# yml-bit/CTA-GAN

Measured on AMD Instinct MI355X. Metric: paired 512x512 slices/sec (G+D step); generator rel-L2 vs CPU reference, higher is better.
Workload: dtype bf16; 1 GPU; HdGan stage-2 full G+D train step (G, Reg, STN, D_m, losses, Adam x3), 16 paired 512x512 slices/GPU; per_gpu_batch=16, global_batch=16, size=512, parallelism=single, rccl_ranks=1, dp_backend=none

## Files before the change

### cta_gan_amd/csrc/conv_wgrad.hip

```cpp
#include <stdlib.h>
#include "conv_dispatch.h"

struct WgradArgs {
    const void* g;
    const void* x;
    float* part;
    int B, Hs, Ws, Mc, g_ld;
    int Hi, Wi, Nc, x_ld;
    int is, pad_mode;
    int slab, sps;
    int ntaps;
    int taps[64];
};

template <typename T> struct WgCfg;
template <> struct WgCfg<bf16_t> { static constexpr int PK = 64, PK_MT = 32, PADB = 32; };
template <> struct WgCfg<float> { static constexpr int PK = 32, PK_MT = 16, PADB = 64; };

template <typename T, int BM, int BN, int NT>
__global__ __launch_bounds__(256) void conv_wgrad_kernel(const WgradArgs a) {
    constexpr int EPC = VecOf<T>::N;
    constexpr int PK = NT > 1 ? WgCfg<T>::PK_MT : WgCfg<T>::PK;
    constexpr int RSM = BM * (int)sizeof(T) + WgCfg<T>::PADB;
    constexpr int RSN = BN * (int)sizeof(T) + WgCfg<T>::PADB;
// ... 899 lines not shown
                h.tmap[cnt++] = t;
            }
            if (cnt == 0) continue;
            const int kh = win.kh(), kw = win.kw();
            ok = cnt == kh * kw;
            for (int i = 0; ok && i < cnt; ++i) {
                const int tw = a.taps[h.tmap[i]];
                const int qy = (tap_dy(tw) - py) / 2, qx = (tap_dx(tw) - px) / 2;
                ok = (qy == win.dy0() + i / kw) && (qx == win.dx0() + i % kw);
            }
            h.g = g; h.x = x; h.part = part;
            h.B = B; h.Hs = Hs; h.Ws = Ws; h.Mc = Mc; h.g_ld = g_ld;
            h.Hi = Hi; h.Wi = Wi; h.Nc = Nc; h.x_ld = x_ld;
            h.pad_mode = pad_mode; h.sps = a.sps; h.ntaps = cnt; h.gtaps = ntaps;
            h.kw = kw; h.khb = kh; h.dy0 = win.dy0(); h.dx0 = win.dx0();
            h.is = 2; h.py = py; h.px = px;
            h.phases = pair ? 3 : 1; h.g_lo = g_ld / 2; h.x_lo = x_ld / 2; h.phase_split = split;
            h.no_reuse = ctg_knobs().wg_no_reuse;
            h.prefetch = !ctg_knobs().wg_noprefetch;
            h.xcd = !ctg_knobs().wg_noxcd;
            const int bm = h.Mc % 64 == 0 ? 64 : h.Mc % 32 == 0 ? 32 : 16, bn = h.Nc % 64 == 0 ? 64 : 32;
            ok = ok && bm >= 32 && !(bm == 32 && bn == 32) && (cnt == 1 || cnt == 2 || cnt == 4) && kw <= 2 && kh <= 2;
            covered += cnt;
            ++nph;
        }
        if (ok && covered == ntaps && ntaps == 9 && nph == 4 && !split) {
            if (taps_3x3(a.taps, false)) {
                WgHaloArgs h = ph[0];
                h.ntaps = 9; h.gtaps = 9; h.kw = 2; h.khb = 2; h.dy0 = -1; h.dx0 = -1; h.py = 0; h.px = 0;
                const int rc = launch_wg_s2m(h, st);
                if (rc != -1) return rc;
            }
        }
        if (ok && covered == ntaps) {
            for (int p = 0; p < nph; ++p) {
                const int rc = launch_wgh_any(ph[p], st);
                if (rc != 0) return rc == -1 ? CTG_EINVAL : rc;
            }
            return split ? 3 : 0;
        }
    }
    if (pair) return 2;
    if (Mc % 32) return CTG_EINVAL;
    return dtype == DT_BF16 ? launch_wg_t<bf16_t>(a, st) : launch_wg_t<float>(a, st);
}

#define RED_MAX_T 24
struct ReduceList {
    const float* part[RED_MAX_T];
    float* dst[RED_MAX_T];
    long sm[RED_MAX_T], sn[RED_MAX_T], stp[RED_MAX_T];
    int Z[RED_MAX_T], ntaps[RED_MAX_T], Mc[RED_MAX_T], Nc[RED_MAX_T], Mreal[RED_MAX_T], Nreal[RED_MAX_T];
    int acc[RED_MAX_T], shift[RED_MAX_T];
    int first[RED_MAX_T + 1];
    int count;
};

__global__ __launch_bounds__(256) void wgrad_reduce_multi_kernel(const ReduceList L) {
    __shared__ float red[256];
    int j = 0;
    while (j + 1 < L.count && (int)blockIdx.x >= L.first[j + 1]) ++j;
    const int shift = L.shift[j], ZP = 1 << shift, IW = 256 >> shift;
    const int il = threadIdx.x & (IW - 1), zq = threadIdx.x >> (8 - shift);
    const int Z = L.Z[j], Mc = L.Mc[j], Nc = L.Nc[j];
    const long E = (long)L.ntaps[j] * Mc * Nc;
    const long idx = (long)((int)blockIdx.x - L.first[j]) * IW + il;
    const float* __restrict__ part = L.part[j];
    float s0 = 0.f, s1 = 0.f, s2 = 0.f, s3 = 0.f;
    if (idx < E) {
        int zz = zq;
        for (; zz + 3 * ZP < Z; zz += 4 * ZP) {
            s0 += part[(long)zz * E + idx];
            s1 += part[(long)(zz + ZP) * E + idx];
            s2 += part[(long)(zz + 2 * ZP) * E + idx];
            s3 += part[(long)(zz + 3 * ZP) * E + idx];
        }
        for (; zz < Z; zz += ZP) s0 += part[(long)zz * E + idx];
    }
    float s = (s0 + s1) + (s2 + s3);
    if (shift) {
        red[zq * IW + il] = s;
        __syncthreads();
        s = 0.f;
        if (zq == 0)
            for (int q = 0; q < ZP; ++q) s += red[q * IW + il];
    }
    if (zq == 0 && idx < E) {
        const int c = (int)(idx % Nc);
        const int m = (int)((idx / Nc) % Mc);
        const int t = (int)(idx / ((long)Nc * Mc));
        if (m < L.Mreal[j] && c < L.Nreal[j]) {
            float* d = L.dst[j] + m * L.sm[j] + c * L.sn[j] + t * L.stp[j];
            *d = L.acc[j] ? *d + s : s;
        }
    }
}

extern "C" int ctg_wgrad_reduce_multi(int count, const void* const* part, void* const* dst, const int* Z,
                                      const int* ntaps, const int* Mc, const int* Nc, const int* Mreal, const int* Nreal,
                                      const long* sm, const long* sn, const long* stp, const int* accumulate,
                                      void* stream) {
    CTG_ENTER();
    if (count < 0) return CTG_EINVAL;
    for (int base = 0; base < count; base += RED_MAX_T) {
        ReduceList L;
        L.count = count - base < RED_MAX_T ? count - base : RED_MAX_T;
        long blocks = 0;
        for (int i = 0; i < L.count; ++i) {
            const int q = base + i;
            if (Z[q] < 1 || ntaps[q] < 1 || Mreal[q] > Mc[q] || Nreal[q] > Nc[q] || part[q] == nullptr || dst[q] == nullptr)
                return CTG_EINVAL;
            const long E = (long)ntaps[q] * Mc[q] * Nc[q];
            const int shift = (Z[q] >= 64 && E <= 65536) ? (E <= 16384 ? 5 : 4) : 0;
            L.part[i] = (const float*)part[q]; L.dst[i] = (float*)dst[q];
            L.sm[i] = sm[q]; L.sn[i] = sn[q]; L.stp[i] = stp[q];
            L.Z[i] = Z[q]; L.ntaps[i] = ntaps[q]; L.Mc[i] = Mc[q]; L.Nc[i] = Nc[q]; L.Mreal[i] = Mreal[q]; L.Nreal[i] = Nreal[q];
            L.acc[i] = accumulate[q]; L.shift[i] = shift;
            L.first[i] = (int)blocks;
            const int iw = 256 >> shift;
            blocks += (E + iw - 1) / iw;
            if (blocks >= (1L << 30)) return CTG_EINVAL;
        }
        L.first[L.count] = (int)blocks;
        if (blocks == 0) continue;
        hipLaunchKernelGGL(wgrad_reduce_multi_kernel, dim3((unsigned)blocks), dim3(256), 0, (hipStream_t)stream, L);
    }
    return ctg_launch_status();
}

extern "C" int ctg_wgrad_reduce(const float* part, int Z, int ntaps, int Mc, int Nc, float* dst, int Mreal, int Nreal,
                                long sm, long sn, long stp, int accumulate, void* stream) {
    CTG_ENTER();
    if (Z < 1 || ntaps < 1 || Mreal > Mc || Nreal > Nc) return CTG_EINVAL;
    const long E = (long)ntaps * Mc * Nc;
    if (Z >= 64 && E <= 65536) {
        if (E <= 16384) {
            hipLaunchKernelGGL(wgrad_reduce_zp_kernel<32>, dim3((unsigned)((E + 7) / 8)), dim3(256), 0,
                               (hipStream_t)stream, part, Z, ntaps, Mc, Nc, dst, Mreal, Nreal, sm, sn, stp, accumulate);
        } else {
            hipLaunchKernelGGL(wgrad_reduce_zp_kernel<16>, dim3((unsigned)((E + 15) / 16)), dim3(256), 0,
                               (hipStream_t)stream, part, Z, ntaps, Mc, Nc, dst, Mreal, Nreal, sm, sn, stp, accumulate);
        }
        return ctg_launch_status();
    }
    const int blocks = (int)((E + 255) / 256 < 4096 ? (E + 255) / 256 : 4096);
    hipLaunchKernelGGL(wgrad_reduce_kernel, dim3(blocks), dim3(256), 0, (hipStream_t)stream, part, Z, ntaps, Mc, Nc,
                       dst, Mreal, Nreal, sm, sn, stp, accumulate);
    return ctg_launch_status();
}
```

### cta_gan_amd/csrc/loss_stn.hip

```cpp
#include "common.h"

static inline int ew_blocks(long items) {
    long b = (items + 255) / 256;
    return (int)(b < 1 ? 1 : (b > 4096 ? 4096 : b));
}

__device__ __forceinline__ void block_partial(float v, float* __restrict__ part) {
    __shared__ float ws[4];
    v = wave_sum(v);
    if ((threadIdx.x & 63) == 0) ws[threadIdx.x >> 6] = v;
    __syncthreads();
    if (threadIdx.x == 0) part[blockIdx.x] = (ws[0] + ws[1]) + (ws[2] + ws[3]);
}

__global__ __launch_bounds__(256) void sum_finalize_kernel(const float* __restrict__ part, int n, float scale,
                                                           float* __restrict__ out, int accumulate) {
    __shared__ double ws[4];
    double s = 0.0;
    for (int i = threadIdx.x; i < n; i += 256) s += (double)part[i];
#pragma unroll
    for (int o = 32; o > 0; o >>= 1) s += __shfl_xor(s, o, 64);
    if ((threadIdx.x & 63) == 0) ws[threadIdx.x >> 6] = s;
    __syncthreads();
    if (threadIdx.x == 0) {
// ... 34 lines not shown
        const float nw = ((fx + 1.f) - ix) * ((fy + 1.f) - iy), ne = (ix - fx) * ((fy + 1.f) - iy);
        const float sw = ((fx + 1.f) - ix) * (iy - fy), se = (ix - fx) * (iy - fy);
        const float* s = src + (size_t)n * H * W;
        float r = s[(size_t)y0 * W + x0] * nw;
        if (x1 < W) r += s[(size_t)y0 * W + x1] * ne;
        if (y1 < H) r += s[(size_t)y1 * W + x0] * sw;
        if (y1 < H && x1 < W) r += s[(size_t)y1 * W + x1] * se;
        out[i] = r;
    }
}

__global__ void zero_f32_kernel(float* __restrict__ p, long n) {
    for (long i = (long)blockIdx.x * blockDim.x + threadIdx.x; i < n; i += (long)gridDim.x * blockDim.x) p[i] = 0.f;
}

__global__ void warp_bwd_kernel(const float* __restrict__ src, const float* __restrict__ flow, long fs_n, long fs_c,
                                long fs_y, long fs_x, const float* __restrict__ gout, float* __restrict__ dsrc,
                                float* __restrict__ dflow, int B, int H, int W) {
    const long total = (long)B * H * W;
    for (long i = (long)blockIdx.x * blockDim.x + threadIdx.x; i < total; i += (long)gridDim.x * blockDim.x) {
        const int x = (int)(i % W);
        const int y = (int)((i / W) % H);
        const int n = (int)(i / ((long)W * H));
        const long fo = n * fs_n + y * fs_y + x * fs_x;
        float iy, ix, my, mx;
        warp_coord((float)y, flow[fo], H, iy, my);
        warp_coord((float)x, flow[fo + fs_c], W, ix, mx);
        const float fy = floorf(iy), fx = floorf(ix);
        const int y0 = (int)fy, x0 = (int)fx, y1 = y0 + 1, x1 = x0 + 1;
        const float wx1 = ix - fx, wx0 = (fx + 1.f) - ix, wy1 = iy - fy, wy0 = (fy + 1.f) - iy;
        const float g = gout[i];
        const float* s = src + (size_t)n * H * W;
        float* ds = dsrc ? dsrc + (size_t)n * H * W : nullptr;
        const bool bx = x1 < W, by = y1 < H;
        const float vnw = s[(size_t)y0 * W + x0];
        const float vne = bx ? s[(size_t)y0 * W + x1] : 0.f;
        const float vsw = by ? s[(size_t)y1 * W + x0] : 0.f;
        const float vse = (bx && by) ? s[(size_t)y1 * W + x1] : 0.f;
        if (ds) {
            atomicAdd(ds + (size_t)y0 * W + x0, wx0 * wy0 * g);
            if (bx) atomicAdd(ds + (size_t)y0 * W + x1, wx1 * wy0 * g);
            if (by) atomicAdd(ds + (size_t)y1 * W + x0, wx0 * wy1 * g);
            if (bx && by) atomicAdd(ds + (size_t)y1 * W + x1, wx1 * wy1 * g);
        }
        if (dflow) {
            const float gix = (-vnw * wy0 + vne * wy0 - vsw * wy1 + vse * wy1) * g;
            const float giy = (-vnw * wx0 - vne * wx1 + vsw * wx0 + vse * wx1) * g;
            dflow[fo] = my * giy;
            dflow[fo + fs_c] = mx * gix;
        }
    }
}

__global__ void warp_det_prep_kernel(const float* __restrict__ gout, long long* __restrict__ acc, unsigned* __restrict__ maxbits,
                                     long n) {
    unsigned m = 0u;
    for (long i = (long)blockIdx.x * blockDim.x + threadIdx.x; i < n; i += (long)gridDim.x * blockDim.x) {
        acc[i] = 0;
        const unsigned b = __float_as_uint(gout[i]) & 0x7fffffffu;
        m = b > m ? b : m;
    }
#pragma unroll
    for (int o = 32; o > 0; o >>= 1) {
        const unsigned t = (unsigned)__shfl_xor((int)m, o, 64);
        m = t > m ? t : m;
    }
    if ((threadIdx.x & 63) == 0 && m) atomicMax(maxbits, m);
}

__device__ __forceinline__ float det_scale(unsigned maxbits, bool inverse) {
    int e = (int)(maxbits >> 23) - 127;
    e = e < -88 ? -88 : (e > 88 ? 88 : e);
    return __uint_as_float((unsigned)((inverse ? e - 38 : 38 - e) + 127) << 23);
}

__global__ void warp_bwd_det_kernel(const float* __restrict__ flow, long fs_n, long fs_c, long fs_y, long fs_x,
                                    const float* __restrict__ gout, long long* __restrict__ acc,
                                    const unsigned* __restrict__ maxbits, int B, int H, int W) {
    const long total = (long)B * H * W;
    const float sc = det_scale(maxbits[0], false);
    for (long i = (long)blockIdx.x * blockDim.x + threadIdx.x; i < total; i += (long)gridDim.x * blockDim.x) {
        const int x = (int)(i % W);
        const int y = (int)((i / W) % H);
        const int n = (int)(i / ((long)W * H));
        const long fo = n * fs_n + y * fs_y + x * fs_x;
        float iy, ix, my, mx;
        warp_coord((float)y, flow[fo], H, iy, my);
        warp_coord((float)x, flow[fo + fs_c], W, ix, mx);
        const float fy = floorf(iy), fx = floorf(ix);
        const int y0 = (int)fy, x0 = (int)fx, y1 = y0 + 1, x1 = x0 + 1;
        const float wx1 = ix - fx, wx0 = (fx + 1.f) - ix, wy1 = iy - fy, wy0 = (fy + 1.f) - iy;
        const float g = gout[i] * sc;
        unsigned long long* ds = reinterpret_cast<unsigned long long*>(acc + (size_t)n * H * W);
        const bool bx = x1 < W, by = y1 < H;
        atomicAdd(ds + (size_t)y0 * W + x0, (unsigned long long)__float2ll_rn(wx0 * wy0 * g));
        if (bx) atomicAdd(ds + (size_t)y0 * W + x1, (unsigned long long)__float2ll_rn(wx1 * wy0 * g));
        if (by) atomicAdd(ds + (size_t)y1 * W + x0, (unsigned long long)__float2ll_rn(wx0 * wy1 * g));
        if (bx && by) atomicAdd(ds + (size_t)y1 * W + x1, (unsigned long long)__float2ll_rn(wx1 * wy1 * g));
    }
}

__global__ void warp_det_finish_kernel(const long long* __restrict__ acc, const unsigned* __restrict__ maxbits,
                                       float* __restrict__ dsrc, long n) {
    const float inv = det_scale(maxbits[0], true);
    for (long i = (long)blockIdx.x * blockDim.x + threadIdx.x; i < n; i += (long)gridDim.x * blockDim.x)
        dsrc[i] = (float)acc[i] * inv;
}

__global__ void smooth_fwd_kernel(const float* __restrict__ f, long sn, long sc, long sy, long sx, int B, int C,
                                  int H, int W, float inv_nx, float inv_ny, float* __restrict__ part) {
    const long total = (long)B * C * H * W;
    float acc = 0.f;
    for (long i = (long)blockIdx.x * blockDim.x + threadIdx.x; i < total; i += (long)gridDim.x * blockDim.x) {
        const int x = (int)(i % W);
        const int y = (int)((i / W) % H);
        const int c = (int)((i / ((long)W * H)) % C);
        const int n = (int)(i / ((long)W * H * C));
        const float* p = f + n * sn + c * sc + y * sy + x * sx;
        const float v = p[0];
        if (x + 1 < W) { const float d = p[sx] - v; acc += d * d * inv_nx; }
// ... 191 lines not shown
    }
    const int t = blockIdx.y;
    if (t >= L.count) return;
    const int n = L.n[t];
    const int beg = blockIdx.x * ADAM_CHUNK;
    if (beg >= n) return;
    const int end = min(beg + ADAM_CHUNK, n);
    float* __restrict__ p = L.p[t];
    const float* __restrict__ g = L.g[t];
    float* __restrict__ m = L.m[t];
    float* __restrict__ v = L.v[t];
    const float step = lr / bc1;
    for (int i = beg + threadIdx.x; i < end; i += 256) {
        const float gi = g[i];
        float mi = m[i], vi = v[i];
        mi = mi + (gi - mi) * (1.f - b1);
        vi = vi * b2 + (1.f - b2) * gi * gi;
        const float denom = sqrtf(vi) / bc2_sqrt + eps;
        p[i] = p[i] - step * (mi / denom);
        m[i] = mi;
        v[i] = vi;
    }
}

__global__ void adam_tick_kernel(float* __restrict__ state, float b1, float b2) {
    if (threadIdx.x == 0 && blockIdx.x == 0) {
        const double step = (double)state[0] + 1.0;
        state[0] = (float)step;
        state[1] = (float)(1.0 - pow((double)b1, step));
        state[2] = (float)sqrt(1.0 - pow((double)b2, step));
    }
}

extern "C" int ctg_warp_fwd(const float* src, const float* flow, long fs_n, long fs_c, long fs_y, long fs_x,
                            float* out, int B, int H, int W, void* stream) {
    CTG_ENTER();
    if (H < 2 || W < 2) return CTG_EINVAL;
    hipLaunchKernelGGL(warp_fwd_kernel, dim3(ew_blocks((long)B * H * W)), dim3(256), 0, (hipStream_t)stream, src,
                       flow, fs_n, fs_c, fs_y, fs_x, out, B, H, W);
    return ctg_launch_status();
}

extern "C" int ctg_warp_bwd(const float* src, const float* flow, long fs_n, long fs_c, long fs_y, long fs_x,
                            const float* gout, float* dsrc, float* dflow, int B, int H, int W, void* det_ws, void* stream) {
    CTG_ENTER();
    if (H < 2 || W < 2) return CTG_EINVAL;
    hipStream_t st = (hipStream_t)stream;
    if (dsrc && det_ws) {
        if ((uintptr_t)det_ws & 7) return CTG_EINVAL;
        const long n = (long)B * H * W;
        long long* acc = (long long*)det_ws;
        unsigned* maxbits = (unsigned*)(acc + n);
        hipLaunchKernelGGL(zero_f32_kernel, dim3(1), dim3(64), 0, st, (float*)maxbits, 2L);
        hipLaunchKernelGGL(warp_det_prep_kernel, dim3(ew_blocks(n)), dim3(256), 0, st, gout, acc, maxbits, n);
        hipLaunchKernelGGL(warp_bwd_det_kernel, dim3(ew_blocks(n)), dim3(256), 0, st, flow, fs_n, fs_c, fs_y, fs_x, gout, acc,
                           maxbits, B, H, W);
        hipLaunchKernelGGL(warp_det_finish_kernel, dim3(ew_blocks(n)), dim3(256), 0, st, acc, maxbits, dsrc, n);
        if (dflow)
            hipLaunchKernelGGL(warp_bwd_kernel, dim3(ew_blocks(n)), dim3(256), 0, st, src, flow, fs_n, fs_c, fs_y, fs_x, gout,
                               (float*)nullptr, dflow, B, H, W);
        return ctg_launch_status();
    }
    if (dsrc) {
        hipLaunchKernelGGL(zero_f32_kernel, dim3(ew_blocks((long)B * H * W / 4 + 1)), dim3(256), 0, st, dsrc, (long)B * H * W);
    }
    hipLaunchKernelGGL(warp_bwd_kernel, dim3(ew_blocks((long)B * H * W)), dim3(256), 0, st, src, flow, fs_n, fs_c,
                       fs_y, fs_x, gout, dsrc, dflow, B, H, W);
    return ctg_launch_status();
}

extern "C" int ctg_smooth_fwd(const float* f, long sn, long sc, long sy, long sx, int B, int C, int H, int W,
                              float weight, float* part, float* out, void* stream) {
    CTG_ENTER();
    if (H < 2 || W < 2) return CTG_EINVAL;
    const long total = (long)B * C * H * W;
    const int nb = ew_blocks(total);
    const float inv_nx = 1.f / (float)((long)B * C * H * (W - 1)), inv_ny = 1.f / (float)((long)B * C * (H - 1) * W);
    hipStream_t st = (hipStream_t)stream;
    hipLaunchKernelGGL(smooth_fwd_kernel, dim3(nb), dim3(256), 0, st, f, sn, sc, sy, sx, B, C, H, W, inv_nx, inv_ny,
                       part);
    hipLaunchKernelGGL(sum_finalize_kernel, dim3(1), dim3(256), 0, st, (const float*)part, nb, weight, out, 0);
    return ctg_launch_status();
}

extern "C" int ctg_smooth_bwd(const float* f, long sn, long sc, long sy, long sx, int B, int C, int H, int W,
                              float weight, const float* gscale, float* df, int accumulate, void* stream) {
    CTG_ENTER();
    if (H < 2 || W < 2) return CTG_EINVAL;
    const long total = (long)B * C * H * W;
    const float inv_nx = weight / (float)((long)B * C * H * (W - 1)), inv_ny = weight / (float)((long)B * C * (H - 1) * W);
    hipLaunchKernelGGL(smooth_bwd_kernel, dim3(ew_blocks(total)), dim3(256), 0, (hipStream_t)stream, f, sn, sc, sy, sx,
                       B, C, H, W, inv_nx, inv_ny, gscale, df, accumulate);
    return ctg_launch_status();
}

extern "C" int ctg_l1_fwd(const float* a, const float* b, const float* mask, long n, float weight, float* part,
                          float* out, void* stream) {
    CTG_ENTER();
    if (n < 1) return CTG_EINVAL;
    const int nb = ew_blocks(n);
    hipStream_t st = (hipStream_t)stream;
    hipLaunchKernelGGL(l1_fwd_kernel, dim3(nb), dim3(256), 0, st, a, b, mask, n, part);
    hipLaunchKernelGGL(sum_finalize_kernel, dim3(1), dim3(256), 0, st, (const float*)part, nb, weight / (float)n, out, 0);
    return ctg_launch_status();
}

extern "C" int ctg_l1_bwd(const float* a, const float* b, const float* mask, long n, float weight, const float* gscale,
// ... 147 lines not shown
```

### cta_gan_amd/csrc/norm_act.hip

```cpp
#include "common.h"
#include "ctg_knobs.h"

#define MAX_SLABS 128

__device__ __forceinline__ int fold_srcs(int y, int H, int p, int* s) {
    int k = 0;
    s[k++] = y;
    if (y >= 1 && y <= p) s[k++] = -y;
    if (y >= H - 1 - p && y <= H - 2) s[k++] = 2 * (H - 1) - y;
    return k;
}

template <typename T>
__device__ __forceinline__ void fold_load(Chunk<T>& out, const T* __restrict__ d, int n, int y, int x, int ch, int H,
                                          int W, int p, int ld) {
    if (p == 0) {
        out.load(d + (((size_t)n * H + y) * W + x) * ld + ch, ld);
        return;
    }
    const int Hp = H + 2 * p, Wp = W + 2 * p;
    int ys[3], xs[3];
    const int ny = fold_srcs(y, H, p, ys), nx = fold_srcs(x, W, p, xs);
    out.zero();
    for (int a = 0; a < ny; ++a)
// ... 44 lines not shown
                    g[u].load(dout + ((size_t)n * HW + pc) * d_ld + ch, d_ld);
                } else {
                    const int y = pc / W;
                    fold_load<T>(g[u], dout, n, y, pc - y * W, ch, H, W, pad, d_ld);
                }
            }
        }
#pragma unroll
        for (int u = 0; u < UNR; ++u) {
            if (!ok[u]) continue;
            if (MODE == 0) {
#pragma unroll
                for (int e = 0; e < EPC; ++e) { s1[e] += v[u].v[e]; s2[e] += v[u].v[e] * v[u].v[e]; }
            } else if (MODE == 1) {
#pragma unroll
                for (int e = 0; e < EPC; ++e) {
                    const float xh = (v[u].v[e] - mu[e]) * rs[e];
                    float gg = g[u].v[e];
                    if (act == ACT_RELU) gg = xh > 0.f ? gg : 0.f;
                    else if (act == ACT_LRELU) gg = xh > 0.f ? gg : LRELU_SLOPE * gg;
                    s1[e] += gg; s2[e] += gg * xh;
                }
            } else if (MODE == 3) {
                Chunk<T> o;
#pragma unroll
                for (int e = 0; e < EPC; ++e) {
                    o.v[e] = g[u].v[e] * act_grad_from_out(v[u].v[e], act);
                    s1[e] += o.v[e];
                }
                o.store(gout + ((size_t)n * HW + pb + u * PL) * go_ld + ch, go_ld);
            } else {
#pragma unroll
                for (int e = 0; e < EPC; ++e) s1[e] += g[u].v[e];
            }
        }
    }
    float* out = part + (((size_t)n * nslabs + slab) * C) * 2;
    __shared__ float stage[256 * 8];
#pragma unroll
    for (int which = 0; which < 2; ++which) {
        __syncthreads();
#pragma unroll
        for (int e = 0; e < EPC; ++e) stage[pl * C + ch + e] = which ? s2[e] : s1[e];
        __syncthreads();
        for (int c = tid; c < C; c += 256) {
            float s = 0.f;
            for (int q = 0; q < PL; ++q) s += stage[q * C + c];
            out[c * 2 + which] = s;
        }
    }
}


__global__ __launch_bounds__(64) void moments_finalize_wave_kernel(const float* __restrict__ part, int nslabs, int C,
                                                                   float invHW, int mode, float* __restrict__ mean,
                                                                   float* __restrict__ rstd) {
    const int i = blockIdx.x;
    const int n = i / C, c = i - n * C;
    double a = 0.0, b = 0.0;
    for (int s = threadIdx.x; s < nslabs; s += 64) {
        const float* p = part + (((size_t)n * nslabs + s) * C + c) * 2;
        a += (double)p[0];
        b += (double)p[1];
    }
#pragma unroll
    for (int o = 32; o > 0; o >>= 1) {
        a += __shfl_xor(a, o, 64);
        b += __shfl_xor(b, o, 64);
    }
    if (threadIdx.x == 0) {
        if (mode == 0) {
            const double m = a * invHW;
            double var = b * invHW - m * m;
            var = var < 0.0 ? 0.0 : var;
            mean[i] = (float)m;
            rstd[i] = (float)(1.0 / sqrt(var + (double)IN_EPS));
        } else {
            mean[i] = (float)(a * invHW);
            rstd[i] = (float)(b * invHW);
        }
    }
}

__global__ __launch_bounds__(64) void bias_finalize_kernel(const float* __restrict__ part, int B, int nslabs, int C,
                                                           int Creal, float* __restrict__ db, int accumulate) {
    const int c = blockIdx.x;
    if (c >= Creal) return;
    const int total = B * nslabs;
    float a = 0.f;
    for (int i = threadIdx.x; i < total; i += 64) a += part[((size_t)i * C + c) * 2];
    a = wave_sum(a);
    if (threadIdx.x == 0) db[c] = accumulate ? db[c] + a : a;
}

template <typename T> struct ChanParams {
    static constexpr int EPC = Chunk<T>::N;
    float v[EPC];
    __device__ __forceinline__ void load(const float* __restrict__ p) {
#pragma unroll
        for (int q = 0; q < EPC / 4; ++q) {
            const f32x4 t = *reinterpret_cast<const f32x4*>(p + 4 * q);
            v[4 * q] = t[0]; v[4 * q + 1] = t[1]; v[4 * q + 2] = t[2]; v[4 * q + 3] = t[3];
        }
    }
};

#define ACT_RT (-1)


template <typename T, int ACT>
__device__ __forceinline__ void in_fwd_px(Chunk<T>& o, const Chunk<T>& v, const ChanParams<T>& mu,
                                          const ChanParams<T>& rs, int act) {
#pragma clang fp contract(off)
#pragma unroll
    for (int e = 0; e < Chunk<T>::N; ++e) {
        const float xh = (v.v[e] - mu.v[e]) * rs.v[e];
        if (ACT == ACT_RT) o.v[e] = act_apply(xh, act);
        else if (ACT == ACT_RELU) o.v[e] = xh > 0.f ? xh : 0.f;
        else if (ACT == ACT_LRELU) o.v[e] = xh > 0.f ? xh : LRELU_SLOPE * xh;
        else o.v[e] = xh;
    }
}

template <typename T> __device__ __forceinline__ void chunk_add(Chunk<T>& o, const Chunk<T>& r) {
#pragma clang fp contract(off)
#pragma unroll
    for (int e = 0; e < Chunk<T>::N; ++e) o.v[e] += r.v[e];
}

template <typename T, typename TX, int ACT>
__device__ __forceinline__ void in_bwd_px(Chunk<T>& o, const Chunk<TX>& v, const Chunk<T>& g, const ChanParams<T>& mu,
                                          const ChanParams<T>& rs, const ChanParams<T>& a1, const ChanParams<T>& a2) {
#pragma unroll
    for (int e = 0; e < Chunk<T>::N; ++e) {
        float inner;
        {
#pragma clang fp contract(off)
            const float xh = (v.v[e] - mu.v[e]) * rs.v[e];
            float gg = g.v[e];
            if (ACT == ACT_RELU) gg = xh > 0.f ? gg : 0.f;
            else if (ACT == ACT_LRELU) gg = xh > 0.f ? gg : LRELU_SLOPE * gg;
            inner = __fmaf_rn(-xh, a2.v[e], gg - a1.v[e]);
        }
        o.v[e] = rs.v[e] * inner;
    }
// ... 392 lines not shown
    switch (act) {
        case ACT_NONE: launch_in_apply_act<T, ACT_NONE>(grid, per, st, x, x_ld, mean, rstd, act, res, r_ld, out, o_ld, HW, C); break;
        case ACT_RELU: launch_in_apply_act<T, ACT_RELU>(grid, per, st, x, x_ld, mean, rstd, act, res, r_ld, out, o_ld, HW, C); break;
        case ACT_LRELU: launch_in_apply_act<T, ACT_LRELU>(grid, per, st, x, x_ld, mean, rstd, act, res, r_ld, out, o_ld, HW, C); break;
        default: launch_in_apply_act<T, ACT_RT>(grid, per, st, x, x_ld, mean, rstd, act, res, r_ld, out, o_ld, HW, C); break;
    }
}
template <typename T, typename TX, int ACT, typename... A>
static inline void launch_in_bwd_apply_act(dim3 grid, int per, hipStream_t st, A... a) {
    constexpr int U = InUnr<TX>::BWD;
    if (U > 2 && per < U) hipLaunchKernelGGL((in_bwd_apply_kernel<T, TX, ACT, 2>), grid, dim3(256), 0, st, a...);
    else hipLaunchKernelGGL((in_bwd_apply_kernel<T, TX, ACT, U>), grid, dim3(256), 0, st, a...);
}
template <typename T, typename TX>
static inline void launch_in_bwd_apply(dim3 grid, int per, hipStream_t st, const TX* x, int x_ld, const T* dout, int d_ld,
                                       int pad, const float* mean, const float* rstd, const float* s1, const float* s2,
                                       int act, T* dx, int dx_ld, int H, int W, int C) {
    switch (act) {
        case ACT_RELU: launch_in_bwd_apply_act<T, TX, ACT_RELU>(grid, per, st, x, x_ld, dout, d_ld, pad, mean, rstd, s1, s2, dx, dx_ld, H, W, C); break;
        case ACT_LRELU: launch_in_bwd_apply_act<T, TX, ACT_LRELU>(grid, per, st, x, x_ld, dout, d_ld, pad, mean, rstd, s1, s2, dx, dx_ld, H, W, C); break;
        default: launch_in_bwd_apply_act<T, TX, ACT_NONE>(grid, per, st, x, x_ld, dout, d_ld, pad, mean, rstd, s1, s2, dx, dx_ld, H, W, C); break;
    }
}

#define DISPATCH_T(dtype, CALL)                   \
    if ((dtype) == DT_BF16) { typedef bf16_t T; CALL; } \
    else if ((dtype) == DT_F32) { typedef float T; CALL; } \
    else if ((dtype) == DT_PAIR) { typedef bfpair_t T; CALL; } \
    else return CTG_EINVAL;

#define DISPATCH_TX(dtype, CALL)                  \
    if ((dtype) == DT_BF16) { typedef bf16_t T; typedef bf16_t TX; CALL; } \
    else if ((dtype) == DT_F32) { typedef float T; typedef float TX; CALL; } \
    else if ((dtype) == DT_PAIR) { typedef bfpair_t T; typedef bfpair_t TX; CALL; } \
    else if ((dtype) == DT_MIX) { typedef bf16_t T; typedef bfpair_t TX; CALL; } \
    else return CTG_EINVAL;

static int check_c(int dtype, int C) {
    const int epc = dtype == DT_F32 ? 4 : 8;
    if (C % epc) return CTG_EINVAL;
    const int cpp = C / epc;
    return (pow2(cpp) && cpp <= 256) ? CTG_OK : CTG_EINVAL;
}

extern "C" int ctg_in_stats(int dtype, const void* x, int x_ld, int B, int H, int W, int C, int nslabs, float* part,
                            float* mean, float* rstd, void* stream) {
    CTG_ENTER();
    if (check_c(dtype, C) || nslabs < 1 || nslabs > MAX_SLABS) return CTG_EINVAL;
    hipStream_t st = (hipStream_t)stream;
    DISPATCH_T(dtype, hipLaunchKernelGGL((moments_partial_kernel<T, 0>), dim3(nslabs, B), dim3(256), 0, st,
                                         (const T*)x, x_ld, (const T*)nullptr, 0, 0, (const float*)nullptr,
                                         (const float*)nullptr, 0, H, W, C, part));
    if (mean != nullptr)
        hipLaunchKernelGGL(moments_finalize_wave_kernel, dim3(B * C), dim3(64), 0, st, part, nslabs, C,
                           1.0f / (float)(H * W), 0, mean, rstd);
    return ctg_launch_status();
}

extern "C" int ctg_in_finalize(const float* part, int B, int C, int nslabs, int HW, int mode, float* mean, float* rstd,
                               void* stream) {
    CTG_ENTER();
    if (B < 1 || C < 1 || nslabs < 1 || HW < 1 || (mode != 0 && mode != 1)) return CTG_EINVAL;
    hipLaunchKernelGGL(moments_finalize_wave_kernel, dim3(B * C), dim3(64), 0, (hipStream_t)stream, part, nslabs, C,
                       1.0f / (float)HW, mode, mean, rstd);
    return ctg_launch_status();
}

extern "C" int ctg_in_apply(int dtype, const void* x, int x_ld, const float* mean, const float* rstd, int act,
                            const void* res, int r_ld, void* out, int o_ld, int B, int H, int W, int C, void* stream) {
    CTG_ENTER();
    if (check_c(dtype, C) || out == nullptr) return CTG_EINVAL;
    int per;
    const dim3 grid = pix_grid(dtype, B, H * W, C, &per);
    DISPATCH_T(dtype, (launch_in_apply<T>(grid, per, (hipStream_t)stream, (const T*)x, x_ld, mean, rstd, act, (const T*)res,
                                          r_ld, (T*)out, o_ld, H * W, C)));
    return ctg_launch_status();
}

static inline dim3 fused_grid(int dtype, int B, int HW, int C, int nslabs, int* cgc_out) {
    const int cpp = C / (dtype == DT_F32 ? 4 : 8);
    const int cgc = cpp < 8 ? cpp : 8;
    const int ncg = cpp / cgc, pl = 256 / cgc;
    long gx = (long)HW / (16L * nslabs);
    if (gx * ncg * B < 1024) gx = (1024 + (long)ncg * B - 1) / ((long)ncg * B);
    const long gmax = ((long)HW + pl * 4 - 1) / (pl * 4);
    if (gx > gmax) gx = gmax;
    if (gx < 1) gx = 1;
    *cgc_out = cgc;
    return dim3((unsigned)gx, (unsigned)ncg, (unsigned)B);
}

extern "C" int ctg_in_apply_part(int dtype, const void* x, int x_ld, const float* part, int nslabs, float* mean,
                                 float* rstd, int act, const void* res, int r_ld, void* out, int o_ld, int B, int H,
                                 int W, int C, void* stream) {
    CTG_ENTER();
    if (check_c(dtype, C) || nslabs < 1 || nslabs > FUSED_MAX_SLABS || part == nullptr || mean == nullptr || rstd == nullptr)
        return CTG_EINVAL;
    int cgc;
    const dim3 grid = fused_grid(dtype, B, H * W, C, nslabs, &cgc);
    DISPATCH_T(dtype, hipLaunchKernelGGL((in_apply_part_kernel<T>), grid, dim3(256), 0, (hipStream_t)stream, (const T*)x,
                                         x_ld, part, nslabs, 1.0f / (float)(H * W), mean, rstd, act, (const T*)res, r_ld,
                                         (T*)out, o_ld, H * W, C, cgc));
    return ctg_launch_status();
}

extern "C" int ctg_in_bwd_partial(int dtype, const void* x, int x_ld, const void* dout, int d_ld, int pad,
                                  const float* mean, const float* rstd, int act, int B, int H, int W, int C, int nslabs,
                                  float* part, void* stream) {
    CTG_ENTER();
    if (check_c(dtype, C) || nslabs < 1 || nslabs > MAX_SLABS || pad < 0 || pad >= H || pad >= W) return CTG_EINVAL;
    DISPATCH_TX(dtype, hipLaunchKernelGGL((moments_partial_kernel<T, 1, TX>), dim3(nslabs, B), dim3(256), 0,
                                          (hipStream_t)stream, (const TX*)x, x_ld, (const T*)dout, d_ld, pad, mean, rstd, act,
                                          H, W, C, part, (T*)nullptr, 0));
    return ctg_launch_status();
}

extern "C" int ctg_in_bwd(int dtype, const void* x, int x_ld, const void* dout, int d_ld, int pad, const float* mean,
// ... 10 lines not shown
                                const float* rstd, const float* s1, const float* s2, int act, void* dx, int dx_ld, int B,
                                int H, int W, int C, void* stream) {
    CTG_ENTER();
    if (check_c(dtype, C) || pad < 0 || pad >= H || pad >= W || s1 == nullptr || s2 == nullptr) return CTG_EINVAL;
    int per;
    const dim3 grid = pix_grid(dtype, B, H * W, C, &per);
    DISPATCH_TX(dtype, (launch_in_bwd_apply<T, TX>(grid, per, (hipStream_t)stream, (const TX*)x, x_ld, (const T*)dout, d_ld,
                                                   pad, mean, rstd, s1, s2, act, (T*)dx, dx_ld, H, W, C)));
    return ctg_launch_status();
}

extern "C" int ctg_in_bwd_stats(int dtype, const void* x, int x_ld, const void* dout, int d_ld, int pad, const float* mean,
                                const float* rstd, int act, void* dx, int dx_ld, int B, int H, int W, int C, int nslabs,
                                const float* part, void* stream) {
    CTG_ENTER();
    if (check_c(dtype, C) || nslabs < 1 || nslabs > FUSED_MAX_SLABS || part == nullptr || pad < 0 || pad >= H || pad >= W)
        return CTG_EINVAL;
    int cgc;
    const dim3 grid = fused_grid(dtype, B, H * W, C, nslabs, &cgc);
    DISPATCH_TX(dtype, hipLaunchKernelGGL((in_bwd_apply_part_kernel<T, TX>), grid, dim3(256), 0, (hipStream_t)stream, (const TX*)x,
                                          x_ld, (const T*)dout, d_ld, pad, mean, rstd, part, nslabs, 1.0f / (float)(H * W), act,
                                          (T*)dx, dx_ld, H, W, C, cgc));
    return ctg_launch_status();
}

extern "C" int ctg_grad_combine(int dtype, const void* a, int a_ld, const void* b, int b_ld, int pad, const void* yact,
                                int y_ld, int act, void* out, int o_ld, int B, int H, int W, int C, void* stream) {
    CTG_ENTER();
    const int epc = dtype == DT_F32 ? 4 : 8;
    if (C % epc || (a == nullptr && b == nullptr) || pad < 0 || pad >= H || pad >= W) return CTG_EINVAL;
    const long items = (long)B * H * W * (C / epc);
    if (items >= (1L << 31)) return CTG_EINVAL;
    DISPATCH_T(dtype, hipLaunchKernelGGL((grad_combine_kernel<T>), dim3(ew_blocks(items)), dim3(256), 0,
                                         (hipStream_t)stream, (const T*)a, a_ld, (const T*)b, b_ld, pad,
                                         (const T*)yact, y_ld, act, (T*)out, o_ld, H, W, C, items));
    return ctg_launch_status();
}

extern "C" int ctg_act_bwd_f32(const float* g, const float* y, int act, float* out, long n, void* stream) {
    CTG_ENTER();
    if (n < 1 || g == nullptr || y == nullptr || out == nullptr) return CTG_EINVAL;
    hipLaunchKernelGGL(act_bwd_f32_kernel, dim3(ew_blocks(n)), dim3(256), 0, (hipStream_t)stream, g, y, act, out, n);
    return ctg_launch_status();
}

extern "C" int ctg_bias_grad(int dtype, const void* g, int g_ld, int pad, int B, int H, int W, int C, int Creal,
                             int nslabs, float* part, float* db, int accumulate, void* stream) {
    CTG_ENTER();
    if (check_c(dtype, C) || nslabs < 1 || nslabs > MAX_SLABS || Creal > C) return CTG_EINVAL;
    hipStream_t st = (hipStream_t)stream;
    DISPATCH_T(dtype, hipLaunchKernelGGL((moments_partial_kernel<T, 2>), dim3(nslabs, B), dim3(256), 0, st,
                                         (const T*)nullptr, 0, (const T*)g, g_ld, pad, (const float*)nullptr,
                                         (const float*)nullptr, 0, H, W, C, part));
    hipLaunchKernelGGL(bias_finalize_kernel, dim3(Creal), dim3(64), 0, st, part, B, nslabs, C, Creal, db,
                       accumulate);
    return ctg_launch_status();
}

extern "C" int ctg_bias_grad_act(int dtype, const void* g, int g_ld, int pad, const void* yact, int y_ld, int act, void* gout,
                                 int go_ld, int B, int H, int W, int C, int Creal, int nslabs, float* part, float* db,
                                 int accumulate, void* stream) {
    CTG_ENTER();
    if (check_c(dtype, C) || nslabs < 1 || nslabs > MAX_SLABS || Creal > C || yact == nullptr || gout == nullptr) return CTG_EINVAL;
    if (act != ACT_RELU && act != ACT_LRELU) return CTG_EINVAL;
    hipStream_t st = (hipStream_t)stream;
    DISPATCH_T(dtype, hipLaunchKernelGGL((moments_partial_kernel<T, 3>), dim3(nslabs, B), dim3(256), 0, st,
                                         (const T*)yact, y_ld, (const T*)g, g_ld, pad, (const float*)nullptr,
                                         (const float*)nullptr, act, H, W, C, part, (T*)gout, go_ld));
    hipLaunchKernelGGL(bias_finalize_kernel, dim3(Creal), dim3(64), 0, st, part, B, nslabs, C, Creal, db, accumulate);
    return ctg_launch_status();
}

extern "C" int ctg_fold_f32(const float* dp, float* out, int B, int H, int W, int C, int pad, void* stream) {
    CTG_ENTER();
    if (pad < 1 || pad >= H || pad >= W || C < 1) return CTG_EINVAL;
    hipLaunchKernelGGL(fold_f32_kernel, dim3(ew_blocks((long)B * H * W * C)), dim3(256), 0, (hipStream_t)stream, dp,
                       out, B, H, W, C, pad);
    return ctg_launch_status();
}
```

Measured before the change: 330.5 slices/s.

## Vectorize and coalesce small reduction and finalize kernels across wgrad, STN, norm

The multi-job wgrad partial reduction now reads float4 vectors when the element count and pointer alignment allow it. The warp determinism prep kernel uses vectorized loads and zeroing, caps its grid, and does a block-level max before a single atomic. The moments and bias finalize kernels switch from one 64-thread block per channel with strided loads to 256-thread blocks covering 16 channels, which coalesces the partial-buffer reads and sums them with a tree reduction. These target memory-bound reduction kernels in the backward pass, at the cost of more code paths and changed summation order.

Measured after the change: 331.2 slices/s, median of 6. No clear change (+0.2%).

```diff
diff --git a/cta_gan_amd/csrc/conv_wgrad.hip b/cta_gan_amd/csrc/conv_wgrad.hip
--- a/cta_gan_amd/csrc/conv_wgrad.hip
+++ b/cta_gan_amd/csrc/conv_wgrad.hip
@@ -975,48 +975,71 @@
     long sm[RED_MAX_T], sn[RED_MAX_T], stp[RED_MAX_T];
     int Z[RED_MAX_T], ntaps[RED_MAX_T], Mc[RED_MAX_T], Nc[RED_MAX_T], Mreal[RED_MAX_T], Nreal[RED_MAX_T];
     int acc[RED_MAX_T], shift[RED_MAX_T];
+    int vec[RED_MAX_T];
     int first[RED_MAX_T + 1];
     int count;
 };
 
-__global__ __launch_bounds__(256) void wgrad_reduce_multi_kernel(const ReduceList L) {
-    __shared__ float red[256];
-    int j = 0;
-    while (j + 1 < L.count && (int)blockIdx.x >= L.first[j + 1]) ++j;
+template <int V> struct RedVec {
+    typedef float __attribute__((ext_vector_type(V))) type;
+    static __device__ __forceinline__ float get(type v, int e) { return v[e]; }
+};
+template <> struct RedVec<1> {
+    typedef float type;
+    static __device__ __forceinline__ float get(float v, int) { return v; }
+};
+
+template <int V>
+__device__ __forceinline__ void wgrad_reduce_job(const ReduceList& L, int j, float* __restrict__ red) {
+    typedef typename RedVec<V>::type fv;
     const int shift = L.shift[j], ZP = 1 << shift, IW = 256 >> shift;
     const int il = threadIdx.x & (IW - 1), zq = threadIdx.x >> (8 - shift);
     const int Z = L.Z[j], Mc = L.Mc[j], Nc = L.Nc[j];
     const long E = (long)L.ntaps[j] * Mc * Nc;
-    const long idx = (long)((int)blockIdx.x - L.first[j]) * IW + il;
+    const long idx = ((long)((int)blockIdx.x - L.first[j]) * IW + il) * V;
     const float* __restrict__ part = L.part[j];
-    float s0 = 0.f, s1 = 0.f, s2 = 0.f, s3 = 0.f;
+    fv s0 = 0.f, s1 = 0.f, s2 = 0.f, s3 = 0.f;
     if (idx < E) {
         int zz = zq;
         for (; zz + 3 * ZP < Z; zz += 4 * ZP) {
-            s0 += part[(long)zz * E + idx];
-            s1 += part[(long)(zz + ZP) * E + idx];
-            s2 += part[(long)(zz + 2 * ZP) * E + idx];
-            s3 += part[(long)(zz + 3 * ZP) * E + idx];
-        }
-        for (; zz < Z; zz += ZP) s0 += part[(long)zz * E + idx];
-    }
-    float s = (s0 + s1) + (s2 + s3);
+            const fv a0 = *reinterpret_cast<const fv*>(part + (long)zz * E + idx);
+            const fv a1 = *reinterpret_cast<const fv*>(part + (long)(zz + ZP) * E + idx);
+            const fv a2 = *reinterpret_cast<const fv*>(part + (long)(zz + 2 * ZP) * E + idx);
+            const fv a3 = *reinterpret_cast<const fv*>(part + (long)(zz + 3 * ZP) * E + idx);
+            s0 += a0; s1 += a1; s2 += a2; s3 += a3;
+        }
+        for (; zz < Z; zz += ZP) s0 += *reinterpret_cast<const fv*>(part + (long)zz * E + idx);
+    }
+    fv s = (s0 + s1) + (s2 + s3);
     if (shift) {
-        red[zq * IW + il] = s;
+        *reinterpret_cast<fv*>(red + (zq * IW + il) * V) = s;
         __syncthreads();
         s = 0.f;
         if (zq == 0)
-            for (int q = 0; q < ZP; ++q) s += red[q * IW + il];
+            for (int q = 0; q < ZP; ++q) s += *reinterpret_cast<const fv*>(red + (q * IW + il) * V);
     }
     if (zq == 0 && idx < E) {
-        const int c = (int)(idx % Nc);
-        const int m = (int)((idx / Nc) % Mc);
-        const int t = (int)(idx / ((long)Nc * Mc));
-        if (m < L.Mreal[j] && c < L.Nreal[j]) {
-            float* d = L.dst[j] + m * L.sm[j] + c * L.sn[j] + t * L.stp[j];
-            *d = L.acc[j] ? *d + s : s;
-        }
-    }
+#pragma unroll
+        for (int e = 0; e < V; ++e) {
+            const long ie = idx + e;
+            const int c = (int)(ie % Nc);
+            const int m = (int)((ie / Nc) % Mc);
+            const int t = (int)(ie / ((long)Nc * Mc));
+            if (m < L.Mreal[j] && c < L.Nreal[j]) {
+                float* d = L.dst[j] + m * L.sm[j] + c * L.sn[j] + t * L.stp[j];
+                const float se = RedVec<V>::get(s, e);
+                *d = L.acc[j] ? *d + se : se;
+            }
+        }
+    }
+}
+
+__global__ __launch_bounds__(256) void wgrad_reduce_multi_kernel(const ReduceList L) {
+    __shared__ __attribute__((aligned(16))) float red[256 * 4];
+    int j = 0;
+    while (j + 1 < L.count && (int)blockIdx.x >= L.first[j + 1]) ++j;
+    if (L.vec[j]) wgrad_reduce_job<4>(L, j, red);
+    else wgrad_reduce_job<1>(L, j, red);
 }
 
 extern "C" int ctg_wgrad_reduce_multi(int count, const void* const* part, void* const* dst, const int* Z,
@@ -1038,9 +1061,10 @@
             L.part[i] = (const float*)part[q]; L.dst[i] = (float*)dst[q];
             L.sm[i] = sm[q]; L.sn[i] = sn[q]; L.stp[i] = stp[q];
             L.Z[i] = Z[q]; L.ntaps[i] = ntaps[q]; L.Mc[i] = Mc[q]; L.Nc[i] = Nc[q]; L.Mreal[i] = Mreal[q]; L.Nreal[i] = Nreal[q];
-            L.acc[i] = accumulate[q]; L.shift[i] = shift;
+            const int vec = (E % 4 == 0 && ((uintptr_t)part[q] & 15) == 0) ? 1 : 0;
+            L.acc[i] = accumulate[q]; L.shift[i] = shift; L.vec[i] = vec;
             L.first[i] = (int)blocks;
-            const int iw = 256 >> shift;
+            const long iw = (long)(256 >> shift) * (vec ? 4 : 1);
             blocks += (E + iw - 1) / iw;
             if (blocks >= (1L << 30)) return CTG_EINVAL;
         }
diff --git a/cta_gan_amd/csrc/loss_stn.hip b/cta_gan_amd/csrc/loss_stn.hip
--- a/cta_gan_amd/csrc/loss_stn.hip
+++ b/cta_gan_amd/csrc/loss_stn.hip
@@ -110,20 +110,48 @@
     }
 }
 
-__global__ void warp_det_prep_kernel(const float* __restrict__ gout, long long* __restrict__ acc, unsigned* __restrict__ maxbits,
-                                     long n) {
+#define WARP_PREP_MAX_BLOCKS 1024
+
+static inline int warp_prep_blocks(long n) {
+    const long b = (n + 1023) / 1024;
+    return (int)(b < 1 ? 1 : (b > WARP_PREP_MAX_BLOCKS ? WARP_PREP_MAX_BLOCKS : b));
+}
+
+__device__ __forceinline__ unsigned abs_bits_max(unsigned m, float g) {
+    const unsigned b = __float_as_uint(g) & 0x7fffffffu;
+    return b > m ? b : m;
+}
+
+__global__ __launch_bounds__(256) void warp_det_prep_kernel(const float* __restrict__ gout, long long* __restrict__ acc,
+                                                            unsigned* __restrict__ maxbits, long n) {
+    __shared__ unsigned wm[4];
     unsigned m = 0u;
-    for (long i = (long)blockIdx.x * blockDim.x + threadIdx.x; i < n; i += (long)gridDim.x * blockDim.x) {
+    const long tid = (long)blockIdx.x * 256 + threadIdx.x, nthr = (long)gridDim.x * 256;
+    const bool vec = (((uintptr_t)gout | (uintptr_t)acc) & 15) == 0;
+    const long n4 = vec ? n / 4 : 0;
+    for (long q = tid; q < n4; q += nthr) {
+        const f32x4 g = *reinterpret_cast<const f32x4*>(gout + 4 * q);
+        longlong2* a = reinterpret_cast<longlong2*>(acc + 4 * q);
+        a[0] = make_longlong2(0, 0);
+        a[1] = make_longlong2(0, 0);
+        m = abs_bits_max(abs_bits_max(abs_bits_max(abs_bits_max(m, g[0]), g[1]), g[2]), g[3]);
+    }
+    for (long i = 4 * n4 + tid; i < n; i += nthr) {
         acc[i] = 0;
-        const unsigned b = __float_as_uint(gout[i]) & 0x7fffffffu;
-        m = b > m ? b : m;
+        m = abs_bits_max(m, gout[i]);
     }
 #pragma unroll
     for (int o = 32; o > 0; o >>= 1) {
         const unsigned t = (unsigned)__shfl_xor((int)m, o, 64);
         m = t > m ? t : m;
     }
-    if ((threadIdx.x & 63) == 0 && m) atomicMax(maxbits, m);
+    if ((threadIdx.x & 63) == 0) wm[threadIdx.x >> 6] = m;
+    __syncthreads();
+    if (threadIdx.x == 0) {
+        const unsigned a = wm[0] > wm[1] ? wm[0] : wm[1], b = wm[2] > wm[3] ? wm[2] : wm[3];
+        m = a > b ? a : b;
+        if (m) atomicMax(maxbits, m);
+    }
 }
 
 __device__ __forceinline__ float det_scale(unsigned maxbits, bool inverse) {
@@ -421,7 +449,7 @@
         long long* acc = (long long*)det_ws;
         unsigned* maxbits = (unsigned*)(acc + n);
         hipLaunchKernelGGL(zero_f32_kernel, dim3(1), dim3(64), 0, st, (float*)maxbits, 2L);
-        hipLaunchKernelGGL(warp_det_prep_kernel, dim3(ew_blocks(n)), dim3(256), 0, st, gout, acc, maxbits, n);
+        hipLaunchKernelGGL(warp_det_prep_kernel, dim3(warp_prep_blocks(n)), dim3(256), 0, st, gout, acc, maxbits, n);
         hipLaunchKernelGGL(warp_bwd_det_kernel, dim3(ew_blocks(n)), dim3(256), 0, st, flow, fs_n, fs_c, fs_y, fs_x, gout, acc,
                            maxbits, B, H, W);
         hipLaunchKernelGGL(warp_det_finish_kernel, dim3(ew_blocks(n)), dim3(256), 0, st, acc, maxbits, dsrc, n);
diff --git a/cta_gan_amd/csrc/norm_act.hip b/cta_gan_amd/csrc/norm_act.hip
--- a/cta_gan_amd/csrc/norm_act.hip
+++ b/cta_gan_amd/csrc/norm_act.hip
@@ -120,45 +120,94 @@
 }
 
 
-__global__ __launch_bounds__(64) void moments_finalize_wave_kernel(const float* __restrict__ part, int nslabs, int C,
-                                                                   float invHW, int mode, float* __restrict__ mean,
-                                                                   float* __restrict__ rstd) {
-    const int i = blockIdx.x;
-    const int n = i / C, c = i - n * C;
-    double a = 0.0, b = 0.0;
-    for (int s = threadIdx.x; s < nslabs; s += 64) {
-        const float* p = part + (((size_t)n * nslabs + s) * C + c) * 2;
-        a += (double)p[0];
-        b += (double)p[1];
-    }
-#pragma unroll
-    for (int o = 32; o > 0; o >>= 1) {
-        a += __shfl_xor(a, o, 64);
-        b += __shfl_xor(b, o, 64);
-    }
-    if (threadIdx.x == 0) {
+#define FIN_CT 16
+#define FIN_ROWS 16
+
+template <typename A>
+__device__ __forceinline__ A fin_tree16(const A* __restrict__ rows) {
+    A v[FIN_ROWS];
+#pragma unroll
+    for (int r = 0; r < FIN_ROWS; ++r) v[r] = rows[r * FIN_CT];
+#pragma unroll
+    for (int o = FIN_ROWS / 2; o > 0; o >>= 1) {
+#pragma unroll
+        for (int r = 0; r < o; ++r) v[r] = v[r] + v[r + o];
+    }
+    return v[0];
+}
+
+__global__ __launch_bounds__(256) void moments_finalize_kernel(const float* __restrict__ part, int nslabs, int C,
+                                                               float invHW, int mode, float* __restrict__ mean,
+                                                               float* __restrict__ rstd) {
+    __shared__ double sa[FIN_ROWS * FIN_CT], sb[FIN_ROWS * FIN_CT];
+    const int ctiles = (C + FIN_CT - 1) / FIN_CT;
+    const int n = blockIdx.x / ctiles, c0 = (blockIdx.x - n * ctiles) * FIN_CT;
+    const int cx = threadIdx.x % FIN_CT, ty = threadIdx.x / FIN_CT;
+    const int c = c0 + cx;
+    double a[4] = {0.0, 0.0, 0.0, 0.0}, b[4] = {0.0, 0.0, 0.0, 0.0};
+    if (c < C) {
+        const float2* __restrict__ p = reinterpret_cast<const float2*>(part) + (size_t)n * nslabs * C + c;
+        for (int s = ty; s < nslabs; s += 64) {
+#pragma unroll
+            for (int q = 0; q < 4; ++q) {
+                const int sq = s + q * FIN_ROWS;
+                if (sq < nslabs) {
+                    const float2 v = p[(size_t)sq * C];
+                    a[q] += (double)v.x;
+                    b[q] += (double)v.y;
+                }
+            }
+        }
+    }
+    sa[ty * FIN_CT + cx] = (a[0] + a[2]) + (a[1] + a[3]);
+    sb[ty * FIN_CT + cx] = (b[0] + b[2]) + (b[1] + b[3]);
+    __syncthreads();
+    if (ty == 0 && c < C) {
+        const double ta = fin_tree16(sa + cx), tb = fin_tree16(sb + cx);
+        const int i = n * C + c;
         if (mode == 0) {
-            const double m = a * invHW;
-            double var = b * invHW - m * m;
+            const double m = ta * invHW;
+            double var = tb * invHW - m * m;
             var = var < 0.0 ? 0.0 : var;
             mean[i] = (float)m;
             rstd[i] = (float)(1.0 / sqrt(var + (double)IN_EPS));
         } else {
-            mean[i] = (float)(a * invHW);
-            rstd[i] = (float)(b * invHW);
-        }
-    }
-}
-
-__global__ __launch_bounds__(64) void bias_finalize_kernel(const float* __restrict__ part, int B, int nslabs, int C,
-                                                           int Creal, float* __restrict__ db, int accumulate) {
-    const int c = blockIdx.x;
-    if (c >= Creal) return;
+            mean[i] = (float)(ta * invHW);
+            rstd[i] = (float)(tb * invHW);
+        }
+    }
+}
+
+static inline void launch_moments_finalize(const float* part, int B, int C, int nslabs, float invHW, int mode, float* mean,
+                                           float* rstd, hipStream_t st) {
+    const int ctiles = (C + FIN_CT - 1) / FIN_CT;
+    hipLaunchKernelGGL(moments_finalize_kernel, dim3((unsigned)(B * ctiles)), dim3(256), 0, st, part, nslabs, C, invHW, mode,
+                       mean, rstd);
+}
+
+__global__ __launch_bounds__(256) void bias_finalize_kernel(const float* __restrict__ part, int B, int nslabs, int C,
+                                                            int Creal, float* __restrict__ db, int accumulate) {
+    __shared__ float sa[FIN_ROWS * FIN_CT];
+    const int cx = threadIdx.x % FIN_CT, ty = threadIdx.x / FIN_CT;
+    const int c = blockIdx.x * FIN_CT + cx;
     const int total = B * nslabs;
-    float a = 0.f;
-    for (int i = threadIdx.x; i < total; i += 64) a += part[((size_t)i * C + c) * 2];
-    a = wave_sum(a);
-    if (threadIdx.x == 0) db[c] = accumulate ? db[c] + a : a;
+    float a[4] = {0.f, 0.f, 0.f, 0.f};
+    if (c < Creal) {
+        const float* __restrict__ p = part + (size_t)c * 2;
+        for (int s = ty; s < total; s += 64) {
+#pragma unroll
+            for (int q = 0; q < 4; ++q) {
+                const int sq = s + q * FIN_ROWS;
+                if (sq < total) a[q] += p[(size_t)sq * C * 2];
+            }
+        }
+    }
+    sa[ty * FIN_CT + cx] = (a[0] + a[2]) + (a[1] + a[3]);
+    __syncthreads();
+    if (ty == 0 && c < Creal) {
+        const float t = fin_tree16(sa + cx);
+        db[c] = accumulate ? db[c] + t : t;
+    }
 }
 
 template <typename T> struct ChanParams {
@@ -657,8 +706,7 @@
                                          (const T*)x, x_ld, (const T*)nullptr, 0, 0, (const float*)nullptr,
                                          (const float*)nullptr, 0, H, W, C, part));
     if (mean != nullptr)
-        hipLaunchKernelGGL(moments_finalize_wave_kernel, dim3(B * C), dim3(64), 0, st, part, nslabs, C,
-                           1.0f / (float)(H * W), 0, mean, rstd);
+        launch_moments_finalize(part, B, C, nslabs, 1.0f / (float)(H * W), 0, mean, rstd, st);
     return ctg_launch_status();
 }
 
@@ -666,8 +714,7 @@
                                void* stream) {
     CTG_ENTER();
     if (B < 1 || C < 1 || nslabs < 1 || HW < 1 || (mode != 0 && mode != 1)) return CTG_EINVAL;
-    hipLaunchKernelGGL(moments_finalize_wave_kernel, dim3(B * C), dim3(64), 0, (hipStream_t)stream, part, nslabs, C,
-                       1.0f / (float)HW, mode, mean, rstd);
+    launch_moments_finalize(part, B, C, nslabs, 1.0f / (float)HW, mode, mean, rstd, (hipStream_t)stream);
     return ctg_launch_status();
 }
 
@@ -784,8 +831,8 @@
     DISPATCH_T(dtype, hipLaunchKernelGGL((moments_partial_kernel<T, 2>), dim3(nslabs, B), dim3(256), 0, st,
                                          (const T*)nullptr, 0, (const T*)g, g_ld, pad, (const float*)nullptr,
                                          (const float*)nullptr, 0, H, W, C, part));
-    hipLaunchKernelGGL(bias_finalize_kernel, dim3(Creal), dim3(64), 0, st, part, B, nslabs, C, Creal, db,
-                       accumulate);
+    hipLaunchKernelGGL(bias_finalize_kernel, dim3((Creal + FIN_CT - 1) / FIN_CT), dim3(256), 0, st, part, B, nslabs, C, Creal,
+                       db, accumulate);
     return ctg_launch_status();
 }
 
@@ -799,7 +846,8 @@
     DISPATCH_T(dtype, hipLaunchKernelGGL((moments_partial_kernel<T, 3>), dim3(nslabs, B), dim3(256), 0, st,
                                          (const T*)yact, y_ld, (const T*)g, g_ld, pad, (const float*)nullptr,
                                          (const float*)nullptr, act, H, W, C, part, (T*)gout, go_ld));
-    hipLaunchKernelGGL(bias_finalize_kernel, dim3(Creal), dim3(64), 0, st, part, B, nslabs, C, Creal, db, accumulate);
+    hipLaunchKernelGGL(bias_finalize_kernel, dim3((Creal + FIN_CT - 1) / FIN_CT), dim3(256), 0, st, part, B, nslabs, C, Creal,
+                       db, accumulate);
     return ctg_launch_status();
 }
 
```
